# BaratiLab/GAMD

Hardware: AMD Instinct MI355X
Metric: atom-steps/sec (force eval + integrate), 10k-atom LJ box (higher is better)
Workload: dtype f32; 1 GPU; C2: 10 000-atom LJ box, rho*=0.5, L=92.29 A, cutoff 3.0 sigma=10.2 A, fp32, 4 conv layers x 128, random-init weights (seed 0), 1 box per GPU; n_atoms=10000, boxes=1, launch=single process

## Files before the change

gamd_amd/csrc/edge_encode.hip:

```cpp
#include "gamd_common.h"
#include "gamd_internal.h"

namespace {

constexpr int ENC_W1_FLOATS = 4 * 6 * 64 * 4;
constexpr int ENC_LDS_FLOATS = ENC_W1_FLOATS + 2 * GAMD_WFRAG_FLOATS + 5 * 128 + 64;

template <int NFEAT, typename CPtr>
__device__ __forceinline__ void edge_features(const EncArgs& a, CPtr cen, int src, int dst, const float4& ps, const float4& pd,
                                              int half, float (&F)[24]) {
#pragma clang fp contract(off)
    const BoxDims B = gamd_edge_box(a, dst);
    const float rx = gamd_min_image_wrapped(ps.x - pd.x, B.bx, B.hx);
    const float ry = gamd_min_image_wrapped(ps.y - pd.y, B.by, B.hy);
    const float rz = gamd_min_image_wrapped(ps.z - pd.z, B.bz, B.hz);
    const float nrm = sqrtf((rx * rx + ry * ry) + rz * rz);
    const float den = nrm + 1e-8f;
    const float d = (nrm - a.length_mean) / a.length_std;
    F[0] = half ? ry / den : rx / den;
    F[1] = half ? d : rz / den;
    if (a.rbf.uniform) {
        gamd_rbf_chains(d, half, a.gamma * -1.4426950408889634f, a.rbf, F);
    } else {
#pragma unroll
// ... 7 lines not shown
        float flag = 0.f;
        if (a.bond_nbr) {
            const int io = a.perm[dst], jo = a.perm[src];
            const int4 nb = *reinterpret_cast<const int4*>(a.bond_nbr + 4 * (size_t)io);
            flag = (nb.x == jo || nb.y == jo || nb.z == jo || nb.w == jo) ? 1.f : 0.f;
        }
        F[22] = half ? 0.f : flag;
    }
}


__device__ __forceinline__ void gelu_block(const f32x16 (&acc)[4], f32x16 (&X)[4], const GeluCoef& k) {
    __builtin_amdgcn_s_setprio(1);
#pragma unroll
    for (int t = 0; t < 4; ++t)
#pragma unroll
        for (int r = 0; r < 16; r += 2) {
            const gelu_f2 y = gelu_pair(gelu_f2{acc[t][r], acc[t][r + 1]}, k);
            X[t][r] = y[0]; X[t][r + 1] = y[1];
        }
    __builtin_amdgcn_s_setprio(0);
}

template <int NFEAT>
__global__ void __launch_bounds__(512, 2) k_edge_encode(EncArgs a) {
    if (a.devflags[DEVFLAG_FROZEN]) return;
    extern __shared__ __attribute__((aligned(16))) float lds[];
    float* w1 = lds;
    float* w2 = w1 + ENC_W1_FLOATS;
    float* w3 = w2 + GAMD_WFRAG_FLOATS;
    float* vb1 = w3 + GAMD_WFRAG_FLOATS;
    float* vb2 = vb1 + 128;
    float* vb3 = vb2 + 128;
    float* vg = vb3 + 128;
    float* vbeta = vg + 128;
    float* cen = vbeta + 128;

    const int tid = threadIdx.x;
    const GeluCoef gk = gelu_coef();
    for (int i = tid; i < ENC_W1_FLOATS / 4; i += 512) ((f32x4*)w1)[i] = ((const f32x4*)a.w1p)[i];
    for (int i = tid; i < GAMD_WFRAG_FLOATS / 4; i += 512) {
        ((f32x4*)w2)[i] = ((const f32x4*)a.w2p)[i];
        ((f32x4*)w3)[i] = ((const f32x4*)a.w3p)[i];
    }
    if (tid < 128) {
        vb1[tid] = a.b1[tid]; vb2[tid] = a.b2[tid]; vb3[tid] = a.b3[tid];
        vg[tid] = a.ln_g[tid]; vbeta[tid] = a.ln_b[tid];
    }
    if (tid < 40) cen[tid] = a.centers[tid];
    __syncthreads();

    const int lane = tid & 63, wave = tid >> 6, slot = lane & 31, half = lane >> 5;
    long long E = a.counters[CNT_E];
    if (E > a.e_cap) E = a.e_cap;
    const int n_tiles = (int)((E + GAMD_TILE - 1) / GAMD_TILE);
    const int n_units = (n_tiles + 3) / 4;
    int first, end, step;
    gamd_xcd_range(n_units, blockIdx.x, gridDim.x, first, end, step);
    const int n_iter = first < end ? ((end - first + step - 1) / step + 1) / 2 : 0;
    auto tile_of = [&](int it) {
        const int u = first + (2 * it + (wave >> 2)) * step;
        return (it < n_iter && u < end) ? u * 4 + (wave & 3) : n_tiles;
    };

    constexpr int KSTEPS = (NFEAT + 1) / 2;

    int E32 = (int)E;
    auto fetch_idx = [&](int tile, int& src, int& dst) -> bool {
        const int x = tile * GAMD_TILE + gamd_pi(slot);
        const bool ok = tile < n_tiles && x < E32;
        const int xc = ok ? x : 0;
        src = GAMD_CHK_RANGE(a.sticky, a.col[xc], 0, a.zero_row, GAMD_CHK_ENC_SRC); dst = GAMD_CHK_RANGE(a.sticky, a.erow[xc], 0, a.zero_row, GAMD_CHK_ENC_DST);
        return ok;
    };
    int src_c, dst_c;
    {
        const bool ok = fetch_idx(tile_of(0), src_c, dst_c);
        src_c = ok ? src_c : 0; dst_c = ok ? dst_c : 0;
    }
    float4 ps = a.pos_s[src_c], pd = a.pos_s[dst_c];

    for (int it = 0; it < n_iter; ++it) {
        const int tile = tile_of(it);
        int src_n, dst_n;
        const bool ok_n = fetch_idx(tile_of(it + 1), src_n, dst_n);
        if (tile >= n_tiles) { asm volatile("" ::"v"(src_n), "v"(dst_n)); continue; }
        const long long x = (long long)tile * GAMD_TILE + gamd_pi(slot);
        const bool valid = x < E;
        const int src = src_c, dst = dst_c;
        float F[24];
        __builtin_amdgcn_s_setprio(1);
        edge_features<NFEAT>(a, cen, src, dst, ps, pd, half, F);
        asm volatile("" : "+v"(F[0]), "+v"(F[23]));
        __builtin_amdgcn_s_setprio(0);
        if (a.feat_dbg && valid) {
#pragma unroll
            for (int s = 0; s < 24; ++s) a.feat_dbg[x * 48 + 2 * s + half] = F[s];
        }

        f32x16 acc[4], X[4];
        load_bias_chain(vb1, half, acc);
#pragma unroll
        for (int tp = 0; tp < 4; ++tp) {
#pragma unroll
            for (int g = 0; g < 6; ++g) {
                if (4 * g >= KSTEPS) break;
                const f32x4 w = ((const f32x4*)w1)[(tp * 6 + g) * 64 + lane];
#pragma unroll
                for (int j = 0; j < 4; ++j)
                    if (4 * g + j < KSTEPS) acc[tp] = mfma32(w[j], F[4 * g + j], acc[tp]);
            }
        }
        gelu_block(acc, X, gk);
        load_bias_chain(vb2, half, acc);
        gemm128<false>((const f32x4*)w2, lane, X, acc);
        gelu_block(acc, X, gk);
        src_c = ok_n ? src_n : 0; dst_c = ok_n ? dst_n : 0;
        ps = a.pos_s[src_c]; pd = a.pos_s[dst_c];
        load_bias_chain(vb3, half, acc);
        gemm128<false>((const f32x4*)w3, lane, X, acc);
        layernorm_chain_centered(acc, vg, vbeta, half, 1e-5f, a.ln_inv_width);
        if (a.self_loop) {
            if (valid && gamd_is_appended_loop(a, x, src, dst)) {
#pragma unroll
                for (int t = 0; t < 4; ++t)
#pragma unroll
                    for (int r = 0; r < 16; ++r) acc[t][r] = 0.f;
            }
        }
        asm volatile("" ::"v"(ps.x), "v"(ps.y), "v"(ps.z), "v"(ps.w), "v"(pd.x), "v"(pd.y), "v"(pd.z), "v"(pd.w));
        f32x4* out = (f32x4*)a.e_frag + (size_t)tile * 16 * 64;
#pragma unroll
        for (int t = 0; t < 4; ++t)
#pragma unroll
            for (int q = 0; q < 4; ++q) {
                f32x4 v;
#pragma unroll
                for (int j = 0; j < 4; ++j) v[j] = acc[t][q * 4 + j];
                out[(t * 4 + q) * 64 + lane] = v;
            }
    }
}

template <int NFEAT>
__global__ void __launch_bounds__(256) k_edge_encode_small(EncArgs a) {
    if (a.devflags[DEVFLAG_FROZEN]) return;
    __shared__ __attribute__((aligned(16))) float xbuf[32 * GAMD_XLD];
    __shared__ float red[4][64];
    const int lane = threadIdx.x & 63, slot = lane & 31, half = lane >> 5;
    const int quarter = __builtin_amdgcn_readfirstlane(threadIdx.x >> 6);
    long long E = a.counters[CNT_E];
    if (E > a.e_cap) E = a.e_cap;
    const int n_tiles = (int)((E + GAMD_TILE - 1) / GAMD_TILE);
    constexpr int KSTEPS = (NFEAT + 1) / 2;

    for (int tile = blockIdx.x; tile < n_tiles; tile += gridDim.x) {
        const long long x = (long long)tile * GAMD_TILE + gamd_pi(slot);
        const bool valid = x < E;
        const int src = valid ? GAMD_CHK_RANGE(a.sticky, a.col[x], 0, a.zero_row, GAMD_CHK_ENC_SRC) : 0, dst = valid ? GAMD_CHK_RANGE(a.sticky, a.erow[x], 0, a.zero_row, GAMD_CHK_ENC_DST) : 0;
        const float4 ps = a.pos_s[src], pd = a.pos_s[dst];
        f32x4 w1[6];
#pragma unroll
        for (int g = 0; g < 6; ++g) w1[g] = ((const f32x4*)a.w1p)[(quarter * 6 + g) * 64 + lane];
        WQuarter wa, wb;
// ... 37 lines not shown
#pragma unroll
        for (int q = 0; q < 4; ++q) {
            f32x4 o;
#pragma unroll
            for (int j = 0; j < 4; ++j) o[j] = zero_row ? 0.f : fmaf(acc[q * 4 + j] * rstd, g[q * 4 + j], b[q * 4 + j]);
            out[(quarter * 4 + q) * 64 + lane] = o;
        }
    }
}

}

int launch_edge_encode_small(const EncArgs& a, int n_blocks, hipStream_t st) {
    if (a.n_feat == 44) hipLaunchKernelGGL((k_edge_encode_small<44>), dim3(n_blocks), dim3(256), 0, st, a);
    else if (a.n_feat == 45) hipLaunchKernelGGL((k_edge_encode_small<45>), dim3(n_blocks), dim3(256), 0, st, a);
    else return -22;
    GAMD_CHECK_LAUNCH();
    return 0;
}

int launch_edge_encode(const EncArgs& a, int n_blocks, hipStream_t st) {
    const size_t lds = sizeof(float) * ENC_LDS_FLOATS;
    static PerDeviceOnce once;
    if (int e = gamd_allow_dynamic_lds(once, (int)lds, k_edge_encode<44>, k_edge_encode<45>)) return e;
    if (a.n_feat == 44) hipLaunchKernelGGL((k_edge_encode<44>), dim3(n_blocks), dim3(512), lds, st, a);
    else if (a.n_feat == 45) hipLaunchKernelGGL((k_edge_encode<45>), dim3(n_blocks), dim3(512), lds, st, a);
    else return -22;
    GAMD_CHECK_LAUNCH();
    return 0;
}
```

gamd_amd/csrc/gamd_api.hip:

```cpp
#include "../../include/gamd_hip.h"
#include "gamd_common.h"
#include "gamd_internal.h"

#include <algorithm>
#include <cmath>
#include <cstdarg>
#include <cstddef>
#include <cstdio>
#include <cstdlib>
#include <cstring>
#include <deque>
#include <map>
#include <string>
#include <vector>

namespace {

thread_local char g_err[512] = "";

int fail(int code, const char* fmt, ...) {
    va_list ap;
    va_start(ap, fmt);
    vsnprintf(g_err, sizeof(g_err), fmt, ap);
    va_end(ap);
// ... 107 lines not shown
    int Dp = 128, DT = 1;
    int norm_bn = 0;
    bool update_edge = false;
    bool node_f16 = false;
    bool wide_enc = false, wide_conv = false;
    bool l0_hoist = false;
    long long small_tile_limit = 512;
    std::map<std::string, HostTensor> host_w;
    bool finalized = false;
    double scaler_mean = 0.0, scaler_var = 1.0;

    DevBuf wblob;
    std::vector<LayerDev> layers;
    const float *enc_w1p = nullptr, *enc_w2p = nullptr, *enc_w3p = nullptr, *enc_b1 = nullptr, *enc_b2 = nullptr,
                *enc_b3 = nullptr, *enc_lng = nullptr, *enc_lnb = nullptr, *centers = nullptr;
    const float *node_emb = nullptr, *nenc_w = nullptr, *nenc_b = nullptr;
    const float *dec_w1p = nullptr, *dec_b1 = nullptr, *dec_w2 = nullptr, *dec_b2 = nullptr;
    float length_mean = 0.f, length_std = 1.f;
    RbfGrid rbf{};

    DevBuf pos_w, pos_s, cell_of, perm, inv_perm, deg, row_ptr, na_excl, bond_nbr;
    DevBuf hbuf, hn, S, D, P, f_norm, f_den;
    DevBuf l0_h, l0_hn, l0_S, l0_D, l0_P;
    DevBuf cell_cnt, cell_fill, cell_start;
    int ncell_cap = 0;
    long long e_cap = 0;
    long long piece_cap = 0;
    DevBuf col, erow, chunk_piece, chunk_mask, e_frag, partial, feat_dbg, e_emb, e_frag2;
    DevBuf counters, tdbg, tmp_eid, ke_partial, com_partial;
    DevBuf cnt2;
    int cnt_parity = 0;
    long long skin_calls = 0;
    int* cur_counters = nullptr;
    int* counters_host = nullptr;
    float* host_in = nullptr;
    float* host_out = nullptr;
    DevBuf pos_in;
    int* sticky_host = nullptr;
    int* sticky_dev = nullptr;
    hipStream_t init_stream = nullptr;
    DevBuf devflags;
    const float* feat_dev = nullptr;
    const uint8_t* rigid_checked = nullptr;
    MdPending pending;
    Reporter rep;
    bool has_bonds = false;
// ... 356 lines not shown
    ea.devflags = h->devflags.as<int>();
    ea.pos_s = h->pos_s.as<float4>();
    ea.col = h->col.as<int>();
    ea.erow = h->erow.as<int>();
    ea.bond_nbr = h->has_bonds ? h->bond_nbr.as<int>() : nullptr;
    ea.perm = h->perm.as<int>();
    ea.row_ptr = h->row_ptr.as<int>();
    ea.self_loop = na.self_loop;
    ea.zero_row = h->n;
    for (int d = 0; d < 3; ++d) { ea.box[d] = h->box[d]; ea.half[d] = 0.5f * h->box[d]; }
    ea.bx = box_ref(h);
    ea.length_mean = h->length_mean;
    ea.length_std = h->length_std;
    ea.gamma = (float)(1.0 / 0.025);
    ea.ln_inv_width = 1.0f / (float)h->Eh_true;
    ea.ln_n_pad = (float)(h->Eh - h->Eh_true);
    ea.n_feat = h->n_feat;
    ea.n_ksteps = (h->n_feat + 1) / 2;
    ea.centers = h->centers;
    ea.rbf = h->rbf;
    ea.w1p = h->enc_w1p; ea.w2p = h->enc_w2p; ea.w3p = h->enc_w3p;
    ea.b1 = h->enc_b1; ea.b2 = h->enc_b2; ea.b3 = h->enc_b3;
    ea.ln_g = h->enc_lng; ea.ln_b = h->enc_lnb;
    ea.e_format = !h->wide_enc ? 0 : h->cfg.edge_dtype == GAMD_EDGE_F16X3 ? 2 : h->cfg.edge_dtype == GAMD_EDGE_BF16 ? 1 : 0;
    ea.e_frag = h->e_frag.as<float>();
    ea.e_cap = h->e_cap;
    ea.sticky = h->sticky_dev;
    ea.feat_dbg = h->cfg.keep_stages ? h->feat_dbg.as<float>() : nullptr;
    int small_tiles = 0;
    if (h->cfg.edge_dtype == GAMD_EDGE_F32) {
        const long long e_est = el ? el->n + (na.self_loop ? h->n : 0)
                                   : (h->counters_host[CNT_E] > 0 ? (long long)h->counters_host[CNT_E] : (long long)((double)h->e_cap / 1.5));
        const long long tiles = (e_est + GAMD_TILE - 1) / GAMD_TILE;
        if (tiles <= h->small_tile_limit) small_tiles = (int)std::max<long long>(1, std::min<long long>(tiles + tiles / 8 + 1, 4096));
    }
    const bool half_quantum = h->wide_conv && h->cfg.edge_dtype == GAMD_EDGE_F32 && (h->cfg.kernel_select & GAMD_KSEL_FORCE_HALF_QUANTUM) != 0;
    bool tev_full = false;
    auto tev_begin = [&](int kind) -> int {
        if (!h->timing) return 0;
        if (h->tev_used + 2 > h->tev.size()) {
            if (h->tev.size() >= 8 * gamd_handle::EVENT_POOL_CAP) { tev_full = true; return 0; }
            for (int k = 0; k < 256; ++k) { hipEvent_t e; HIP_TRY(hipEventCreate(&e)); h->tev.push_back(e); h->tev_kind.push_back(0); }
        }
        h->tev_kind[h->tev_used] = kind;
        HIP_TRY(hipEventRecord(h->tev[h->tev_used], st));
        return 0;
// ... 36 lines not shown
    no.piece_cap = h->piece_cap;
    no.P_in = h->P.as<float>();
    no.hn_perm = (!h->wide_conv && h->cfg.edge_dtype == GAMD_EDGE_F16X3) ? 1 : 0;
    no.tab16 = (!h->wide_conv && h->cfg.edge_dtype == GAMD_EDGE_BF16) ? 1 : 0;
    no.hn_out = h->hn.as<float>(); no.S_out = h->S.as<float>(); no.D_out = h->D.as<float>(); no.P_out = h->P.as<float>();
    no.dec_w1p = h->dec_w1p; no.dec_b1 = h->dec_b1; no.dec_w2 = h->dec_w2; no.dec_b2 = h->dec_b2;
    no.ln_inv_width = 1.0f / (float)h->H_true;
    no.ln_n_pad = (float)(h->H - h->H_true);
    no.norm_bn = h->norm_bn;
    no.f16x3 = h->node_f16 ? 1 : 0;
    no.scale = (float)std::sqrt(h->scaler_var);
    no.shift = (float)h->scaler_mean;
    no.perm = h->perm.as<int>();
    no.forces_norm = out_norm_dev ? out_norm_dev : h->f_norm.as<float>();
    no.forces = out_denorm_dev;

    const bool l0 = h->skin > 0.f && !el;
    float* const h0 = (l0 && !h->cfg.keep_stages) ? h->l0_h.as<float>() : hptr(0);
    no.mode = 0;
    no.pre = h->layers[0].node;
    no.h_out = h0;
    if (l0) { no.hn_out = h->l0_hn.as<float>(); no.S_out = h->l0_S.as<float>(); no.D_out = h->l0_D.as<float>(); no.P_out = h->l0_P.as<float>(); }
    no.l0_gate = (l0 && l0_reuse) ? 1 : 0;
    if ((r = node(no))) return fail(-1, "node(0) launch failed (%d)", r);
    no.l0_gate = 0;
    no.hn_out = h->hn.as<float>(); no.S_out = h->S.as<float>(); no.D_out = h->D.as<float>(); no.P_out = h->P.as<float>();
    mark("node_first");


    for (int l = 0; l < h->L; ++l) {
        ConvEdgeArgs ca{};
        ca.counters = h->cur_counters;
        ca.devflags = h->devflags.as<int>();
        ca.col = h->col.as<int>(); ca.erow = h->erow.as<int>();
        ca.chunk_piece = h->chunk_piece.as<int>(); ca.chunk_mask = h->chunk_mask.as<unsigned>();
        ca.e_frag = (h->update_edge && l > 0) ? h->e_frag2.as<float>() : h->e_frag.as<float>();
        ca.emb_out = (h->update_edge && l + 1 < h->L) ? h->e_emb.as<float>() : nullptr;
        ca.hn = h->hn.as<float>(); ca.S = h->S.as<float>(); ca.D = h->D.as<float>();
        if (l0 && l == 0) { ca.hn = h->l0_hn.as<float>(); ca.S = h->l0_S.as<float>(); ca.D = h->l0_D.as<float>(); }
        const LayerDev& ld = h->layers[l];
        ca.w1p = ld.w1p; ca.w2p = ld.w2p; ca.w3p = ld.w3p; ca.w4p = ld.w4p; ca.w16p = ld.w16p;
        ca.b1 = ld.b1; ca.b3 = ld.b3; ca.b4 = ld.b4;
        const bool hoist = l == 0 && h->l0_hoist;
        if (hoist) { ca.w3p = ld.w3p_l0; ca.b3 = ld.b3_l0; }
        ca.partial = h->partial.as<float>();
        ca.piece_cap = h->piece_cap;
        ca.sticky = h->sticky_dev;
        ca.e_cap = h->e_cap;
// ... 211 lines not shown
#ifdef GAMD_CHECKED
const char* gamd_version(void) { return "gamd_hip 0.1 (gfx950) checked"; }
#else
const char* gamd_version(void) { return "gamd_hip 0.1 (gfx950)"; }
#endif
const char* gamd_last_error(void) { return g_err; }

int32_t gamd_create(const gamd_config* cfg, gamd_handle** out) {
    if (!cfg || !out) return fail(-22, "null argument");
    if (cfg->n_atoms <= 0) return fail(-22, "n_atoms must be positive");
    if (cfg->n_boxes < 0 || cfg->n_boxes > (1 << 20)) return fail(-22, "n_boxes out of range");
    const int n_boxes = cfg->n_boxes > 1 ? cfg->n_boxes : 1;
    if ((long long)cfg->n_atoms * n_boxes >= (1 << 23) - 1)
        return fail(-22, "n_atoms x n_boxes = %lld: at most %d atoms per handle", (long long)cfg->n_atoms * n_boxes, (1 << 23) - 2);
    if (cfg->n_layers <= 0 || cfg->n_layers > 16) return fail(-22, "n_layers out of range");
    if (!(cfg->cutoff > 0.f)) return fail(-22, "cutoff must be positive");
    if (cfg->edge_dtype != GAMD_EDGE_F32 && cfg->edge_dtype != GAMD_EDGE_BF16 && cfg->edge_dtype != GAMD_EDGE_F16X3)
        return fail(-22, "unknown edge_dtype");
    if (!(cfg->neighbor_skin >= 0.f)) return fail(-22, "neighbor_skin must be >= 0");
    if (cfg->self_loop_mode != GAMD_SELF_LOOP_DGL07_NOOP && cfg->self_loop_mode != GAMD_SELF_LOOP_APPEND_ZERO_FEATURE)
        return fail(-22, "unknown self_loop_mode %d", cfg->self_loop_mode);
    if (cfg->self_loop_mode != GAMD_SELF_LOOP_DGL07_NOOP && cfg->edge_dtype != GAMD_EDGE_F32)
        return fail(-22, "self_loop_mode 1 is built for the fp32 edge dtype only");
    if (cfg->kernel_select & ~(GAMD_KSEL_FORCE_GENERIC_WIDTH | GAMD_KSEL_FORCE_HALF_QUANTUM | GAMD_KSEL_NO_LAYER0_HOIST))
        return fail(-22, "unknown kernel_select bits 0x%x", cfg->kernel_select);
    int ndev = 0;
    if (hipGetDeviceCount(&ndev) != hipSuccess || ndev <= 0)
        return fail(-19, "no HIP device available: libgamd_hip has no CPU fallback");
    if (cfg->device < 0 || cfg->device >= ndev) return fail(-22, "device %d out of range (%d visible)", cfg->device, ndev);
    DeviceGuard guard(cfg->device);
    hipDeviceProp_t prop;
    HIP_TRY(hipGetDeviceProperties(&prop, cfg->device));
    const int H_true = cfg->encoding_size ? cfg->encoding_size : 128, Eh_true = cfg->edge_embedding_dim ? cfg->edge_embedding_dim : 128;
    const int D_true = cfg->hidden_dim ? cfg->hidden_dim : 128;
    if (H_true < 1 || H_true > 256 || Eh_true < 1 || Eh_true > 256)
        return fail(-22, "encoding_size and edge_embedding_dim must be in [1, 256] (got %d, %d)", H_true, Eh_true);
    if (D_true < 1 || D_true > 256) return fail(-22, "hidden_dim must be in [1, 256] (got %d)", D_true);
    const int Dp = D_true <= 128 ? 128 : 256;
    if (Dp > 128 && cfg->edge_dtype != GAMD_EDGE_F32)
        return fail(-22, "hidden_dim above 128 is built for edge_dtype f32 only (got hidden_dim %d)", D_true);
    const int H = H_true <= 128 ? 128 : 256, Eh = Eh_true <= 128 ? 128 : 256;
    const bool exact128 = H_true == 128 && Eh_true == 128 && D_true == 128;
    const bool generic = H != 128 || Eh != 128 || cfg->no_expand_edge;
    if (cfg->edge_dtype != GAMD_EDGE_F32 && H == 256 && (long long)cfg->n_atoms * n_boxes > (1ll << 22) - 2)
        return fail(-22, "bf16 / split-fp16 with encoding_size > 128: at most 2^22 - 2 atoms per handle (32-bit byte offsets into hn)");
    gamd_handle* h = new gamd_handle();
    h->cfg = *cfg;
// ... 450 lines not shown
        LayerDev& d = h->layers[l];
        d.w1p = B + o.w1p; d.w2p = B + o.w2p; d.w3p = B + o.w3p; d.w4p = B + o.w4p;
        d.w16p = (h->wide_conv && h->cfg.edge_dtype == GAMD_EDGE_F32 && DT == 1) ? B + o.w16p : nullptr;
        d.b1 = B + o.b1; d.b3 = B + o.b3; d.b4 = B + o.b4;
        d.node.ln_g = B + o.lng; d.node.ln_b = B + o.lnb;
        if (update_edge) { d.e_ln_g = B + o.elng; d.e_ln_b = B + o.elnb; }
        d.node.wsp = B + o.wsp; d.node.wdp = B + o.wdp; d.node.wpdp = B + o.wpdp;
        d.node.bS = B + o.bS; d.node.bP = B + o.bP;
        d.node.wpep = B + o.wpep; d.node.wphip = B + o.wphip; d.node.bphi = B + o.bphi;
        d.node.c0 = nullptr;
        if (l == 0 && h->l0_hoist) {
            d.w3p_l0 = B + o.w3p_l0; d.b3_l0 = B + o.b3_l0;
            d.node.wpep = B + o.m0; d.node.c0 = B + o.c0;
        }
    }
    h->enc_w1p = B + o_e1; h->enc_w2p = B + o_e2; h->enc_w3p = B + o_e3;
    h->enc_b1 = B + o_eb1; h->enc_b2 = B + o_eb2; h->enc_b3 = B + o_eb3;
    h->enc_lng = B + o_elg; h->enc_lnb = B + o_elb; h->centers = B + o_cen;
    h->dec_w1p = B + o_d1; h->dec_b1 = B + o_db1; h->dec_w2 = B + o_d2; h->dec_b2 = B + o_db2;
    h->node_emb = h->cfg.kind == GAMD_KIND_LJ ? B + o_emb : nullptr;
    h->nenc_w = h->cfg.kind == GAMD_KIND_LJ ? nullptr : B + o_nw;
    h->nenc_b = h->cfg.kind == GAMD_KIND_LJ ? nullptr : B + o_nb;
    h->finalized = true;
    return 0;
}

int32_t gamd_set_scaler(gamd_handle* h, double mean, double var) {
    if (!h) return fail(-22, "null handle");
    if (!(var >= 0.0)) return fail(-22, "scaler variance must be non-negative");
    h->scaler_mean = mean;
    h->scaler_var = var;
    return 0;
}

int32_t gamd_set_bonds(gamd_handle* h, const int32_t* bonds, int64_t n_bonds) {
    if (!h || (!bonds && n_bonds > 0)) return fail(-22, "bad argument to gamd_set_bonds");
    DeviceGuard guard(h->dev);
    InitStream init(h->init_stream);
    std::vector<int> tab((size_t)h->n * 4, -1);
    auto add = [&](int i, int j) -> int {
        for (int k = 0; k < 4; ++k) {
            if (tab[(size_t)i * 4 + k] == j) return 0;
            if (tab[(size_t)i * 4 + k] < 0) { tab[(size_t)i * 4 + k] = j; return 0; }
        }
        return -1;
    };
    for (int box = 0; box < h->n_boxes; ++box)
        for (int64_t b = 0; b < n_bonds; ++b) {
            int i = bonds[2 * b], j = bonds[2 * b + 1];
            if (i < 0 || j < 0 || i >= h->n_per_box || j >= h->n_per_box)
                return fail(-22, "bond %lld references atom out of range", (long long)b);
            i += box * h->n_per_box; j += box * h->n_per_box;
            if (add(i, j) || add(j, i)) return fail(-22, "more than 4 bonded partners for one atom is not supported");
        }
    if (h->bond_nbr.ensure(sizeof(int) * tab.size(), false)) return fail(-12, "bond table allocation failed");
    HIP_TRY(init_upload(h->bond_nbr.p, tab.data(), sizeof(int) * tab.size()));
    h->has_bonds = n_bonds > 0;
    return 0;
}

int32_t gamd_set_node_features(gamd_handle* h, const float* feat_dev) {
    if (!h) return fail(-22, "null handle");
    if (feat_dev && h->cfg.kind != GAMD_KIND_WATER) return fail(-22, "node features belong to the water models (the LJ model has node_emb)");
    h->feat_dev = feat_dev;
    return 0;
}

int32_t gamd_get_device_flags(gamd_handle* h, int32_t flags[4]) {
    if (!h || !flags) return fail(-22, "null argument");
    flags[0] = h->sticky_host[STICKY_NONFINITE] ? 1 : 0;
    flags[1] = flags[2] = flags[3] = 0;
    h->sticky_host[STICKY_NONFINITE] = 0;
    return 0;
}

int32_t gamd_build_neighbors(gamd_handle* h, const float* pos_dev, const uint8_t* species_dev, const float* box, void* stream) {
    int r;
    if ((r = check_ready(h))) return r;
    if (!pos_dev || !box) return fail(-22, "null argument");
    DeviceGuard guard(h->dev);
    InitStream init((hipStream_t)stream);
    hipStream_t st = (hipStream_t)stream;
    for (int attempt = 0; attempt < 4; ++attempt) {
        if ((r = set_box(h, box, st))) return r;
        h->cur_counters = h->counters.as<int>();
        NbrArgs na = nbr_args(h, pos_dev, species_dev);
        h->cand_valid = false;
// ... 490 lines not shown
```

gamd_amd/csrc/gamd_internal.h:

```cpp
#pragma once
#include <hip/hip_runtime.h>
#include <stdint.h>
#include <atomic>
#include "gamd_common.h"

enum { CNT_E = 0, CNT_PIECES = 1, CNT_OVERFLOW = 2, CNT_TILES = 3, CNT_REBUILD = 4, CNT_NCAND = 5,
       CNT_CAND_MAX = 6,
       CNT_COUNT = 8 };
enum { STICKY_EDGE_OVERFLOW = 0, STICKY_CAND_OVERFLOW = 1, STICKY_REBUILDS = 2, STICKY_NCAND = 3,
       STICKY_NONFINITE = 4,
       STICKY_CHECK_CODE = 5, STICKY_CHECK_VALUE = 6, STICKY_CHECK_LINE = 7,
       STICKY_COUNT = 8 };
enum { GAMD_CHK_CELL = 101, GAMD_CHK_CAND = 102, GAMD_CHK_EDGE_POS = 103, GAMD_CHK_PERM = 104, GAMD_CHK_ENC_SRC = 111, GAMD_CHK_ENC_DST = 112,
       GAMD_CHK_CONV_SRC = 121, GAMD_CHK_CONV_DST = 122, GAMD_CHK_PIECE = 123, GAMD_CHK_NODE_PIECES = 131, GAMD_CHK_INJECTED = 199 };
#ifdef GAMD_CHECKED
template <typename T>
__device__ __forceinline__ T gamd_chk_range(int* sticky, T v, long long lo, long long hi, int code, int line) {
    if ((long long)v >= lo && (long long)v <= hi) return v;
    if (sticky && sticky[STICKY_CHECK_CODE] == 0) {
        sticky[STICKY_CHECK_VALUE] = (int)v;
        sticky[STICKY_CHECK_LINE] = line;
        __threadfence_system();
        sticky[STICKY_CHECK_CODE] = code;
    }
// ... 101 lines not shown
    const int* erow;
    const int* bond_nbr;
    const int* perm;
    const int* row_ptr;
    int self_loop;
    int zero_row;
    float box[3], half[3];
    BoxRef bx;
    float length_mean, length_std, gamma;
    float ln_inv_width, ln_n_pad;
    int n_feat;
    int n_ksteps;
    const float* centers;
    RbfGrid rbf;
    const float* w1p;
    const float* w2p;
    const float* w3p;
    const float* b1; const float* b2; const float* b3;
    const float* ln_g; const float* ln_b;
    float* e_frag;
    long long e_cap;
    float* feat_dbg;
    int* sticky;
    int e_format;
};
__device__ __forceinline__ bool gamd_is_appended_loop(const EncArgs& a, long long x, int src, int dst) {
    if (!a.self_loop || src == a.zero_row) return false;
    const long long row_end = a.row_ptr[dst + 1];
    return x == row_end - 1 || (x + 1 < row_end && a.col[x + 1] == a.zero_row);
}

__device__ __forceinline__ BoxDims gamd_edge_box(const EncArgs& a, int dst) {
    return gamd_box_dims(a.bx, a.box, a.half, a.bx.n_boxes > 1 ? gamd_box_of(a.bx, dst) : 0);
}
int launch_edge_encode(const EncArgs& a, int n_blocks, hipStream_t st);
int launch_edge_encode_small(const EncArgs& a, int n_blocks, hipStream_t st);
int launch_edge_encode_bf16(const EncArgs& a, int n_blocks, hipStream_t st);
int launch_edge_encode_f16x3(const EncArgs& a, int n_blocks, hipStream_t st);
int launch_edge_encode_wide(const EncArgs& a, int eht, int n_blocks, hipStream_t st);
int launch_edge_encode_wide_d(const EncArgs& a, int eht, int dt, int n_blocks, hipStream_t st);

struct ConvEdgeArgs {
    const int* counters;
    const int* devflags;
    const int* col;
    const int* erow;
// ... 35 lines not shown
    const float* ln_g; const float* ln_b;
    float ln_inv_width, ln_n_pad;
    float* e_frag_out;
};
int launch_edge_update(const EdgeUpdateArgs& a, int ht, int n_blocks, hipStream_t st);

struct NodeLayerW {
    const float* ln_g; const float* ln_b;
    const float* wsp; const float* wdp; const float* wpdp;
    const float* bS;
    const float* bP;
    const float* wpep;
    const float* c0;
    const float* wphip;
    const float* bphi;
};
struct NodeArgs {
    const int* counters;
    const int* devflags;
    int* sticky;
    int n;
    int mode;
    int l0_gate;
    const float4* pos_s;
    const float* node_emb;
    const float* enc_w; const float* enc_b;
    const int* row_ptr; const int* na_excl; const int* deg;
    const int* col;
    const float* partial;
    long long piece_cap;
    const float* h_in;
    const float* P_in;
    NodeLayerW post;
    NodeLayerW pre;
    const float* dec_w1p; const float* dec_b1; const float* dec_w2; const float* dec_b2;
    float scale, shift;
    float ln_inv_width, ln_n_pad;
    int norm_bn;
    int f16x3;
    const int* perm;
    float* h_out;
    float* hn_out; float* S_out; float* D_out; float* P_out;
    int hn_perm;
    int tab16;
    float* forces_norm;
    float* forces;
// ... 92 lines not shown
```

gamd_amd/csrc/node.hip:

```cpp
#include "gamd_common.h"
#include "gamd_internal.h"

namespace {

typedef _Float16 nf16x8 __attribute__((ext_vector_type(8)));
typedef _Float16 nf16x2 __attribute__((ext_vector_type(2)));
typedef float nf32x2 __attribute__((ext_vector_type(2)));

constexpr int NT = 16;
constexpr int XLD = 136;

__device__ __forceinline__ f32x4 mfma16(float a, float b, f32x4 c) {
    return __builtin_amdgcn_mfma_f32_16x16x4f32(a, b, c, 0, 0, 0);
}

struct WHalf { f32x4 w[8]; };
__device__ __forceinline__ void load_whalf(const float* __restrict__ Wp, int w, int lane, int half, WHalf& h) {
    const f32x4* W = reinterpret_cast<const f32x4*>(Wp) + (size_t)w * 16 * 64 + lane;
#pragma unroll
    for (int o = 0; o < 2; ++o)
#pragma unroll
        for (int b = 0; b < 4; ++b) h.w[o * 4 + b] = W[(o * 8 + 4 * half + b) * 64];
}

// ... 76 lines not shown
    const nf16x2 lo = __builtin_convertvector(nf32x2{v[0], v[1]}, nf16x2), hi = __builtin_convertvector(nf32x2{v[2], v[3]}, nf16x2);
    return nf16x4{lo[0], lo[1], hi[0], hi[1]};
}
__device__ __forceinline__ void store16_h(_Float16* __restrict__ row, int w, int g, const f32x4 (&v)[2]) {
    *reinterpret_cast<nf16x4*>(row + 32 * w + 4 * g) = cvt16x4(v[0]);
    *reinterpret_cast<nf16x4*>(row + 32 * w + 16 + 4 * g) = cvt16x4(v[1]);
}
__device__ __forceinline__ void store16_tab(_Float16* __restrict__ row, int w, int g, const f32x4 (&v)[2]) {
    *reinterpret_cast<nf16x4*>(row + 32 * w + 8 * (g & 1) + 4 * (g >> 1)) = cvt16x4(v[0]);
    *reinterpret_cast<nf16x4*>(row + 32 * w + 16 + 8 * (g & 1) + 4 * (g >> 1)) = cvt16x4(v[1]);
}

__device__ __forceinline__ float group_sum(float v) {
    v += __shfl_xor(v, 16, 64);
    return v + __shfl_xor(v, 32, 64);
}

template <bool F16>
__global__ void __launch_bounds__(256, 3) k_node(NodeArgs a) {
    __shared__ __attribute__((aligned(16))) float xbuf[NT * XLD];
    __shared__ float obuf[4][NT][3];
    __shared__ float red[2][4][NT];

    if (a.counters[CNT_OVERFLOW] || a.devflags[DEVFLAG_FROZEN]) return;
    if (a.mode == 0 && a.l0_gate && a.counters[CNT_REBUILD] == 0) return;

    const int lane = threadIdx.x & 63, la = lane & 15, g = lane >> 4;
    const int w = __builtin_amdgcn_readfirstlane(threadIdx.x >> 6);
    const int atom_raw = blockIdx.x * NT + la;
    const bool valid = atom_raw < a.n;
    const int atom = valid ? atom_raw : a.n - 1;
    const size_t row = (size_t)atom * GAMD_H;

#ifdef GAMD_PROFILING
    long long tm[16] = {0, 0, 0, 0, 0, 0, 0, 0, 0, 0, 0, 0, 0, 0, 0, 0};
#define NMARK(I) do { if (a.tdbg) tm[I] = (long long)__builtin_readcyclecounter(); } while (0)
#else
#define NMARK(I) do { } while (0)
#endif
    NMARK(0);
    f32x4 XB[8];
    XSplit XS;
#define GEMM16(NEXT, W, NXT) do { if constexpr (F16) gemm16<NEXT, true>(W, NXT, wn, XS, mine, w, lane); \
                                  else gemm16<NEXT, false>(W, NXT, wn, XB, mine, w, lane); } while (0)
#define SPLIT16() do { if constexpr (F16) split16(XB, XS); } while (0)
    f32x4 mine[2];
    WHalf wn;
// ... 203 lines not shown
```

gamd_amd/csrc/wide.hip:

```cpp
#include "gamd_common.h"
#include "gamd_bf16.h"
#include "gamd_f16x3.h"
#include "gamd_internal.h"
#include "gamd_wide.h"

namespace {

constexpr int WIDE_ENC_W1_FLOATS = 4 * 6 * 64 * 4;

__device__ __forceinline__ void wide_barrier() {
    asm volatile("s_waitcnt vmcnt(0) lgkmcnt(0)" ::: "memory");
    __builtin_amdgcn_s_barrier();
    asm volatile("" ::: "memory");
}

template <int EHT> struct EncWaves { static constexpr int value = EHT == 2 ? 4 : 8; };

template <int NFEAT, int EHT, bool LP = false>
__global__ void __launch_bounds__(64 * EncWaves<EHT>::value) k_edge_encode_wide(EncArgs a) {
    if (a.devflags[DEVFLAG_FROZEN]) return;
    static_assert(EHT == 1 || EHT == 2, "edge embedding width 128 or 256");
    constexpr int EH = 128 * EHT;
    constexpr int NW = EncWaves<EHT>::value, NT = 64 * NW;
    constexpr bool EXPAND = NFEAT >= 44;
// ... 375 lines not shown
    for (int i = 0; i < 8; ++i) { o.w[i] = W[i * 64]; o.w[8 + i] = W[2048 + i * 64]; }
}
__device__ __forceinline__ void wq_gemm_f16(const WQ& wq, const f32x16 (&X)[4], f32x16& acc) {
#pragma unroll
    for (int t = 0; t < 4; ++t)
#pragma unroll
        for (int u = 0; u < 2; ++u) {
            f16x8 xh, xl;
            gamd_split8(X[t], u, xh, xl);
            const f16x8 wh = __builtin_bit_cast(f16x8, wq.w[t * 2 + u]), wl = __builtin_bit_cast(f16x8, wq.w[8 + t * 2 + u]);
            acc = mfma_f16(wh, xl, acc);
            acc = mfma_f16(wl, xh, acc);
            acc = mfma_f16(wh, xh, acc);
        }
}
template <int HT, bool F16 = false>
__global__ void __launch_bounds__(256) k_node_wide(NodeArgs a) {
    constexpr int H = 128 * HT;
    constexpr int XLDW = H + 4;
    __shared__ __attribute__((aligned(16))) float xbuf[32 * XLDW];
    __shared__ float obuf[4][32][3];
    __shared__ float red[2][4][32];

    if (a.counters[CNT_OVERFLOW] || a.devflags[DEVFLAG_FROZEN]) return;
    if (a.mode == 0 && a.l0_gate && a.counters[CNT_REBUILD] == 0) return;

    const int lane = threadIdx.x & 63, slot = lane & 31, half = lane >> 5;
    const int quarter = __builtin_amdgcn_readfirstlane(threadIdx.x >> 6);
    const int atom_raw = blockIdx.x * GAMD_TILE + slot;
    const bool valid = atom_raw < a.n;
    const int atom = valid ? atom_raw : a.n - 1;
    const size_t rowH = (size_t)atom * H, rowD = (size_t)atom * 128;

    f32x16 X[HT][4];
    f32x16 mine[HT];
    WQ wqa, wqb;
    constexpr size_t BLK = GAMD_WFRAG_FLOATS;
    auto wptr = [&](int st) -> const float* {
        if (st < HT) return a.post.wpep + (size_t)st * BLK;
        if (st < 2 * HT) return a.post.wphip + (size_t)(st - HT) * BLK;
        const int i = st - 2 * HT;
        if (a.mode == 2) return i < HT ? a.dec_w1p + (size_t)i * BLK : nullptr;
        if (i < HT) return a.pre.wsp + (size_t)i * BLK;
        if (i < 2 * HT) return a.pre.wdp + (size_t)(i - HT) * BLK;
        return i < 3 * HT ? a.pre.wpdp + (size_t)(i - 2 * HT) * BLK : nullptr;
    };
    auto step = [&](int st, const f32x16 (&Xb)[4], f32x16& acc) {
// ... 230 lines not shown
```

gamd_amd/csrc/wide_d.hip:

```cpp
#include "gamd_common.h"
#include "gamd_internal.h"
#include "gamd_wide.h"

namespace {

constexpr int ENC_W1_BLOCK_FLOATS = 4 * 6 * 64 * 4;

__device__ __forceinline__ void wd_barrier() {
    asm volatile("s_waitcnt vmcnt(0) lgkmcnt(0)" ::: "memory");
    __builtin_amdgcn_s_barrier();
    asm volatile("" ::: "memory");
}

template <int NP>
struct BlockRing {
    const float* blocks;
    float* lds;
    int wave;
    unsigned lane16;
    unsigned g = 0;
    int blk = 0;
    __device__ __forceinline__ void prime() { gamd_stage_weight_raw_contig<4>(blocks, lds, wave, lane16); }
    __device__ __forceinline__ const f32x4* begin() {
        const int nb = (blk + 1 == NP) ? 0 : blk + 1;
// ... 319 lines not shown
                                    for (int k = 1; k < 16; ++k) v = (r == k) ? U[tp][k] : v;
                                    a.partial[(size_t)p * H + 128 * ob + 32 * tp + slot] = v;
                                }
                                ++p;
                            }
                        }
                    }
                }
                ring.end();
            }
        }
    }
}


template <int HT, int DT>
__global__ void __launch_bounds__(256) k_node_wide_d(NodeArgs a) {
    constexpr int H = 128 * HT, DP = 128 * DT, NB = HT * DT;
    constexpr int XLDW = 128 * (HT > DT ? HT : DT) + 4;
    __shared__ __attribute__((aligned(16))) float xbuf[32 * XLDW];
    __shared__ float obuf[4][32][3];
    __shared__ float red[2][4][32];

    if (a.counters[CNT_OVERFLOW] || a.devflags[DEVFLAG_FROZEN]) return;
    if (a.mode == 0 && a.l0_gate && a.counters[CNT_REBUILD] == 0) return;

    const int lane = threadIdx.x & 63, slot = lane & 31, half = lane >> 5;
    const int quarter = __builtin_amdgcn_readfirstlane(threadIdx.x >> 6);
    const int atom_raw = blockIdx.x * GAMD_TILE + slot;
    const bool valid = atom_raw < a.n;
    const int atom = valid ? atom_raw : a.n - 1;
    const size_t rowH = (size_t)atom * H, rowD = (size_t)atom * DP;

    f32x16 XH[HT][4];
    f32x16 mine[HT];
    WQ wqa, wqb;
    constexpr size_t BLK = GAMD_WFRAG_FLOATS;
    auto wptr = [&](int st) -> const float* {
        if (st < NB) return a.post.wpep + (size_t)st * BLK;
        if (st < 2 * NB) return a.post.wphip + (size_t)(st - NB) * BLK;
        const int i = st - 2 * NB;
        if (a.mode == 2) return i < NB ? a.dec_w1p + (size_t)i * BLK : nullptr;
        if (i < NB) return a.pre.wsp + (size_t)i * BLK;
        if (i < 2 * NB) return a.pre.wdp + (size_t)(i - NB) * BLK;
        return i < 3 * NB ? a.pre.wpdp + (size_t)(i - 2 * NB) * BLK : nullptr;
    };
    auto step = [&](int st, const f32x16 (&Xb)[4], f32x16& acc) {
// ... 233 lines not shown
```

gamd_amd/engine.py:

```python
from __future__ import annotations

import ctypes as C
from typing import Dict, Optional, Sequence, Tuple, Union

import numpy as np
import torch

from . import _lib
from ._lib import GamdReportParams, GamdConfig, GamdMdParams, GamdNhcParams, check
from .weights import ModelConfig, infer_config, validate_state_dict

ArrayLike = Union[np.ndarray, torch.Tensor]

KIND = {"lj": 0, "water": 1, "dynbox": 1}
FLAVOUR = {"jaxmd": 0, "torch": 1}
SELF_LOOP = {"dgl07_noop": 0, "append_zero_feature_loops": 1}
KSEL_FORCE_GENERIC_WIDTH = 1
KSEL_NO_LAYER0_HOIST = 4


def _box3(box) -> np.ndarray:
    b = np.asarray(box, dtype=np.float64).reshape(-1)
    if b.size == 1:
        b = np.repeat(b, 3)
    if b.size != 3:
        raise ValueError("box must be a scalar or 3 values")
    return b.astype(np.float32)


def _boxes(box, n_boxes: int) -> np.ndarray:
    b = np.asarray(box, dtype=np.float64)
    if b.ndim == 0 or b.size == 1 or (b.ndim == 1 and b.size == 3):
        return np.tile(_box3(b), (n_boxes, 1))
    if b.ndim == 2 and b.shape == (n_boxes, 3):
        return b.astype(np.float32)
    if (b.ndim == 1 and b.size == n_boxes) or (b.ndim == 2 and b.shape == (n_boxes, 1)):
        return np.repeat(b.reshape(-1).astype(np.float32)[:, None], 3, axis=1)
    raise ValueError(f"box must be a scalar, 3 values, [{n_boxes}, 1] or [{n_boxes}, 3] ({n_boxes} boxes)")


class RunReport:
# ... 447 lines not shown
```

include/gamd_hip.h:

```cpp
#ifndef GAMD_HIP_H
#define GAMD_HIP_H

#include <stdint.h>
#include <stddef.h>

#ifdef __cplusplus
extern "C" {
#endif

typedef struct gamd_handle gamd_handle;

enum { GAMD_EDGE_F32 = 0, GAMD_EDGE_BF16 = 1, GAMD_EDGE_F16X3 = 2 };

enum { GAMD_KIND_LJ = 0, GAMD_KIND_WATER = 1 };
enum { GAMD_NBR_JAXMD = 0, GAMD_NBR_TORCH = 1 };

typedef struct gamd_config {
    int32_t n_atoms;
    int32_t kind;
    int32_t n_layers;
    int32_t use_bond;
    int32_t nbr_flavour;
    int32_t device;
    float cutoff;
    float box[3];
    int64_t edge_capacity;
    int32_t keep_stages;
    int32_t edge_dtype;
    int32_t encoding_size;
    int32_t edge_embedding_dim;
    int32_t hidden_dim;
    int32_t no_expand_edge;
    float neighbor_skin;
    int32_t self_loop_mode;
    int32_t kernel_select;
    int32_t small_tile_limit;
    int32_t n_boxes;
} gamd_config;
enum { GAMD_SELF_LOOP_DGL07_NOOP = 0, GAMD_SELF_LOOP_APPEND_ZERO_FEATURE = 1 };
enum { GAMD_KSEL_FORCE_GENERIC_WIDTH = 1, GAMD_KSEL_FORCE_HALF_QUANTUM = 2, GAMD_KSEL_NO_LAYER0_HOIST = 4 };

const char* gamd_version(void);
const char* gamd_last_error(void);

int32_t gamd_create(const gamd_config* cfg, gamd_handle** out);
int32_t gamd_destroy(gamd_handle* h);

int32_t gamd_load_weight(gamd_handle* h, const char* name, const float* data, const int64_t* shape, int32_t ndim);
int32_t gamd_finalize_weights(gamd_handle* h);

int32_t gamd_set_scaler(gamd_handle* h, double mean, double var);

int32_t gamd_set_bonds(gamd_handle* h, const int32_t* bonds, int64_t n_bonds);

int32_t gamd_forces_async(gamd_handle* h, const float* pos_dev, const uint8_t* species_dev, const float* box,
                          float* out_norm_dev, float* out_denorm_dev, void* stream);

int32_t gamd_set_node_features(gamd_handle* h, const float* feat_dev);

int32_t gamd_sync_status(gamd_handle* h, void* stream);

int32_t gamd_get_device_flags(gamd_handle* h, int32_t flags[4]);

// ... 93 lines not shown
```

Baseline: 3.371 million atom-steps/s.

## Overlap encoder weight staging with first tile; cache constant layer-0 node table

```diff
diff --git a/gamd_amd/csrc/edge_encode.hip b/gamd_amd/csrc/edge_encode.hip
--- a/gamd_amd/csrc/edge_encode.hip
+++ b/gamd_amd/csrc/edge_encode.hip
@@ -1,3 +1,4 @@
+#include <type_traits>
 #include "gamd_common.h"
 #include "gamd_internal.h"
 
@@ -53,7 +54,14 @@
     __builtin_amdgcn_s_setprio(0);
 }
 
-template <int NFEAT>
+template <int N>
+__device__ __forceinline__ void weights_landed() {
+    asm volatile("s_waitcnt vmcnt(%0) lgkmcnt(0)" ::"n"(N) : "memory");
+    __builtin_amdgcn_s_barrier();
+    asm volatile("" ::: "memory");
+}
+
+template <int NFEAT, bool OVERLAP>
 __global__ void __launch_bounds__(512, 2) k_edge_encode(EncArgs a) {
     if (a.devflags[DEVFLAG_FROZEN]) return;
     extern __shared__ __attribute__((aligned(16))) float lds[];
@@ -69,19 +77,8 @@
 
     const int tid = threadIdx.x;
     const GeluCoef gk = gelu_coef();
-    for (int i = tid; i < ENC_W1_FLOATS / 4; i += 512) ((f32x4*)w1)[i] = ((const f32x4*)a.w1p)[i];
-    for (int i = tid; i < GAMD_WFRAG_FLOATS / 4; i += 512) {
-        ((f32x4*)w2)[i] = ((const f32x4*)a.w2p)[i];
-        ((f32x4*)w3)[i] = ((const f32x4*)a.w3p)[i];
-    }
-    if (tid < 128) {
-        vb1[tid] = a.b1[tid]; vb2[tid] = a.b2[tid]; vb3[tid] = a.b3[tid];
-        vg[tid] = a.ln_g[tid]; vbeta[tid] = a.ln_b[tid];
-    }
-    if (tid < 40) cen[tid] = a.centers[tid];
-    __syncthreads();
-
-    const int lane = tid & 63, wave = tid >> 6, slot = lane & 31, half = lane >> 5;
+    const int lane = tid & 63, slot = lane & 31, half = lane >> 5;
+    const int wave = __builtin_amdgcn_readfirstlane(tid >> 6);
     long long E = a.counters[CNT_E];
     if (E > a.e_cap) E = a.e_cap;
     const int n_tiles = (int)((E + GAMD_TILE - 1) / GAMD_TILE);
@@ -104,18 +101,53 @@
         src = GAMD_CHK_RANGE(a.sticky, a.col[xc], 0, a.zero_row, GAMD_CHK_ENC_SRC); dst = GAMD_CHK_RANGE(a.sticky, a.erow[xc], 0, a.zero_row, GAMD_CHK_ENC_DST);
         return ok;
     };
+    auto stage_small = [&]() {
+        for (int i = tid; i < ENC_W1_FLOATS / 4; i += 512) ((f32x4*)w1)[i] = ((const f32x4*)a.w1p)[i];
+        if (tid < 128) {
+            vb1[tid] = a.b1[tid]; vb2[tid] = a.b2[tid]; vb3[tid] = a.b3[tid];
+            vg[tid] = a.ln_g[tid]; vbeta[tid] = a.ln_b[tid];
+        }
+        if (tid < 40) cen[tid] = a.centers[tid];
+    };
+    constexpr bool overlap = OVERLAP;
+    if (overlap && n_iter == 0) return;
     int src_c, dst_c;
-    {
+    float4 ps, pd;
+    if (overlap) {
         const bool ok = fetch_idx(tile_of(0), src_c, dst_c);
         src_c = ok ? src_c : 0; dst_c = ok ? dst_c : 0;
+        ps = a.pos_s[src_c]; pd = a.pos_s[dst_c];
+        stage_small();
+        asm volatile("s_waitcnt vmcnt(0)" ::"v"(ps.x), "v"(ps.y), "v"(ps.z), "v"(ps.w), "v"(pd.x), "v"(pd.y), "v"(pd.z), "v"(pd.w) : "memory");
+        gamd_stage_weight_raw_contig<8>(a.w2p, w2, wave, (unsigned)lane * 16u);
+        gamd_stage_weight_raw_contig<8>(a.w3p, w3, wave, (unsigned)lane * 16u);
+        asm volatile("s_waitcnt lgkmcnt(0)" ::: "memory");
+        __builtin_amdgcn_s_barrier();
+        asm volatile("" ::: "memory");
+    } else {
+        stage_small();
+        for (int i = tid; i < GAMD_WFRAG_FLOATS / 4; i += 512) {
+            ((f32x4*)w2)[i] = ((const f32x4*)a.w2p)[i];
+            ((f32x4*)w3)[i] = ((const f32x4*)a.w3p)[i];
+        }
+        __syncthreads();
+        const bool ok = fetch_idx(tile_of(0), src_c, dst_c);
+        src_c = ok ? src_c : 0; dst_c = ok ? dst_c : 0;
+        ps = a.pos_s[src_c]; pd = a.pos_s[dst_c];
     }
-    float4 ps = a.pos_s[src_c], pd = a.pos_s[dst_c];
-
-    for (int it = 0; it < n_iter; ++it) {
+
+    auto iteration = [&](int it, auto first_tag) __attribute__((always_inline)) {
+        constexpr bool landing = OVERLAP && decltype(first_tag)::value;
+        int half_v = half;
+        asm volatile("" : "+v"(half_v));
         const int tile = tile_of(it);
         int src_n, dst_n;
         const bool ok_n = fetch_idx(tile_of(it + 1), src_n, dst_n);
-        if (tile >= n_tiles) { asm volatile("" ::"v"(src_n), "v"(dst_n)); continue; }
+        if (tile >= n_tiles) {
+            asm volatile("" ::"v"(src_n), "v"(dst_n));
+            if (landing) { weights_landed<0>(); weights_landed<0>(); }
+            return;
+        }
         const long long x = (long long)tile * GAMD_TILE + gamd_pi(slot);
         const bool valid = x < E;
         const int src = src_c, dst = dst_c;
@@ -130,7 +162,7 @@
         }
 
         f32x16 acc[4], X[4];
-        load_bias_chain(vb1, half, acc);
+        load_bias_chain(vb1, half_v, acc);
 #pragma unroll
         for (int tp = 0; tp < 4; ++tp) {
 #pragma unroll
@@ -143,14 +175,16 @@
             }
         }
         gelu_block(acc, X, gk);
-        load_bias_chain(vb2, half, acc);
+        if (landing) weights_landed<8>();
+        load_bias_chain(vb2, half_v, acc);
         gemm128<false>((const f32x4*)w2, lane, X, acc);
         gelu_block(acc, X, gk);
+        if (landing) weights_landed<0>();
         src_c = ok_n ? src_n : 0; dst_c = ok_n ? dst_n : 0;
         ps = a.pos_s[src_c]; pd = a.pos_s[dst_c];
-        load_bias_chain(vb3, half, acc);
+        load_bias_chain(vb3, half_v, acc);
         gemm128<false>((const f32x4*)w3, lane, X, acc);
-        layernorm_chain_centered(acc, vg, vbeta, half, 1e-5f, a.ln_inv_width);
+        layernorm_chain_centered(acc, vg, vbeta, half_v, 1e-5f, a.ln_inv_width);
         if (a.self_loop) {
             if (valid && gamd_is_appended_loop(a, x, src, dst)) {
 #pragma unroll
@@ -170,7 +204,10 @@
                 for (int j = 0; j < 4; ++j) v[j] = acc[t][q * 4 + j];
                 out[(t * 4 + q) * 64 + lane] = v;
             }
-    }
+    };
+    int it0 = 0;
+    if (OVERLAP) { iteration(0, std::true_type{}); it0 = 1; }
+    for (int it = it0; it < n_iter; ++it) iteration(it, std::false_type{});
 }
 
 template <int NFEAT>
@@ -254,9 +291,11 @@
 int launch_edge_encode(const EncArgs& a, int n_blocks, hipStream_t st) {
     const size_t lds = sizeof(float) * ENC_LDS_FLOATS;
     static PerDeviceOnce once;
-    if (int e = gamd_allow_dynamic_lds(once, (int)lds, k_edge_encode<44>, k_edge_encode<45>)) return e;
-    if (a.n_feat == 44) hipLaunchKernelGGL((k_edge_encode<44>), dim3(n_blocks), dim3(512), lds, st, a);
-    else if (a.n_feat == 45) hipLaunchKernelGGL((k_edge_encode<45>), dim3(n_blocks), dim3(512), lds, st, a);
+    if (int e = gamd_allow_dynamic_lds(once, (int)lds, k_edge_encode<44, true>, k_edge_encode<45, true>, k_edge_encode<44, false>, k_edge_encode<45, false>)) return e;
+    if (a.n_feat == 44 && a.stage_overlap) hipLaunchKernelGGL((k_edge_encode<44, true>), dim3(n_blocks), dim3(512), lds, st, a);
+    else if (a.n_feat == 44) hipLaunchKernelGGL((k_edge_encode<44, false>), dim3(n_blocks), dim3(512), lds, st, a);
+    else if (a.n_feat == 45 && a.stage_overlap) hipLaunchKernelGGL((k_edge_encode<45, true>), dim3(n_blocks), dim3(512), lds, st, a);
+    else if (a.n_feat == 45) hipLaunchKernelGGL((k_edge_encode<45, false>), dim3(n_blocks), dim3(512), lds, st, a);
     else return -22;
     GAMD_CHECK_LAUNCH();
     return 0;
diff --git a/gamd_amd/csrc/gamd_api.hip b/gamd_amd/csrc/gamd_api.hip
--- a/gamd_amd/csrc/gamd_api.hip
+++ b/gamd_amd/csrc/gamd_api.hip
@@ -153,6 +153,7 @@
     DevBuf pos_w, pos_s, cell_of, perm, inv_perm, deg, row_ptr, na_excl, bond_nbr;
     DevBuf hbuf, hn, S, D, P, f_norm, f_den;
     DevBuf l0_h, l0_hn, l0_S, l0_D, l0_P;
+    bool l0_written = false;
     DevBuf cell_cnt, cell_fill, cell_start;
     int ncell_cap = 0;
     long long e_cap = 0;
@@ -555,6 +556,7 @@
     ea.w1p = h->enc_w1p; ea.w2p = h->enc_w2p; ea.w3p = h->enc_w3p;
     ea.b1 = h->enc_b1; ea.b2 = h->enc_b2; ea.b3 = h->enc_b3;
     ea.ln_g = h->enc_lng; ea.ln_b = h->enc_lnb;
+    ea.stage_overlap = (h->cfg.kernel_select & GAMD_KSEL_NO_ENC_OVERLAP) ? 0 : 1;
     ea.e_format = !h->wide_enc ? 0 : h->cfg.edge_dtype == GAMD_EDGE_F16X3 ? 2 : h->cfg.edge_dtype == GAMD_EDGE_BF16 ? 1 : 0;
     ea.e_frag = h->e_frag.as<float>();
     ea.e_cap = h->e_cap;
@@ -637,8 +639,18 @@
     no.h_out = h0;
     if (l0) { no.hn_out = h->l0_hn.as<float>(); no.S_out = h->l0_S.as<float>(); no.D_out = h->l0_D.as<float>(); no.P_out = h->l0_P.as<float>(); }
     no.l0_gate = (l0 && l0_reuse) ? 1 : 0;
-    if ((r = node(no))) return fail(-1, "node(0) launch failed (%d)", r);
+    bool l0_cache = l0 && !h->cfg.keep_stages && h->node_emb && !h->feat_dev && !(h->cfg.kernel_select & GAMD_KSEL_NO_L0_TABLE_CACHE);
+    if (l0_cache && !h->l0_written) {
+        hipStreamCaptureStatus cs = hipStreamCaptureStatusNone;
+        if (hipStreamIsCapturing(st, &cs) != hipSuccess || cs != hipStreamCaptureStatusNone) l0_cache = false;
+    }
+    if (!(l0_cache && h->l0_written)) {
+        if (l0_cache) { no.l0_gate = 0; no.l0_const = 1; }
+        if ((r = node(no))) return fail(-1, "node(0) launch failed (%d)", r);
+        if (l0_cache) h->l0_written = true;
+    }
     no.l0_gate = 0;
+    no.l0_const = 0;
     no.hn_out = h->hn.as<float>(); no.S_out = h->S.as<float>(); no.D_out = h->D.as<float>(); no.P_out = h->P.as<float>();
     mark("node_first");
 
@@ -896,7 +908,8 @@
         return fail(-22, "unknown self_loop_mode %d", cfg->self_loop_mode);
     if (cfg->self_loop_mode != GAMD_SELF_LOOP_DGL07_NOOP && cfg->edge_dtype != GAMD_EDGE_F32)
         return fail(-22, "self_loop_mode 1 is built for the fp32 edge dtype only");
-    if (cfg->kernel_select & ~(GAMD_KSEL_FORCE_GENERIC_WIDTH | GAMD_KSEL_FORCE_HALF_QUANTUM | GAMD_KSEL_NO_LAYER0_HOIST))
+    if (cfg->kernel_select & ~(GAMD_KSEL_FORCE_GENERIC_WIDTH | GAMD_KSEL_FORCE_HALF_QUANTUM | GAMD_KSEL_NO_LAYER0_HOIST |
+                               GAMD_KSEL_NO_L0_TABLE_CACHE | GAMD_KSEL_NO_ENC_OVERLAP))
         return fail(-22, "unknown kernel_select bits 0x%x", cfg->kernel_select);
     int ndev = 0;
     if (hipGetDeviceCount(&ndev) != hipSuccess || ndev <= 0)
@@ -1393,6 +1406,7 @@
     h->nenc_w = h->cfg.kind == GAMD_KIND_LJ ? nullptr : B + o_nw;
     h->nenc_b = h->cfg.kind == GAMD_KIND_LJ ? nullptr : B + o_nb;
     h->finalized = true;
+    h->l0_written = false;
     return 0;
 }
 
@@ -1434,6 +1448,7 @@
     if (!h) return fail(-22, "null handle");
     if (feat_dev && h->cfg.kind != GAMD_KIND_WATER) return fail(-22, "node features belong to the water models (the LJ model has node_emb)");
     h->feat_dev = feat_dev;
+    h->l0_written = false;
     return 0;
 }
 
diff --git a/gamd_amd/csrc/gamd_internal.h b/gamd_amd/csrc/gamd_internal.h
--- a/gamd_amd/csrc/gamd_internal.h
+++ b/gamd_amd/csrc/gamd_internal.h
@@ -147,6 +147,7 @@
     long long e_cap;
     float* feat_dbg;
     int* sticky;
+    int stage_overlap;
     int e_format;
 };
 __device__ __forceinline__ bool gamd_is_appended_loop(const EncArgs& a, long long x, int src, int dst) {
@@ -228,6 +229,7 @@
     int n;
     int mode;
     int l0_gate;
+    int l0_const;
     const float4* pos_s;
     const float* node_emb;
     const float* enc_w; const float* enc_b;
diff --git a/gamd_amd/csrc/node.hip b/gamd_amd/csrc/node.hip
--- a/gamd_amd/csrc/node.hip
+++ b/gamd_amd/csrc/node.hip
@@ -122,7 +122,7 @@
     __shared__ float obuf[4][NT][3];
     __shared__ float red[2][4][NT];
 
-    if (a.counters[CNT_OVERFLOW] || a.devflags[DEVFLAG_FROZEN]) return;
+    if (!(a.mode == 0 && a.l0_const) && (a.counters[CNT_OVERFLOW] || a.devflags[DEVFLAG_FROZEN])) return;
     if (a.mode == 0 && a.l0_gate && a.counters[CNT_REBUILD] == 0) return;
 
     const int lane = threadIdx.x & 63, la = lane & 15, g = lane >> 4;
diff --git a/gamd_amd/csrc/wide.hip b/gamd_amd/csrc/wide.hip
--- a/gamd_amd/csrc/wide.hip
+++ b/gamd_amd/csrc/wide.hip
@@ -421,7 +421,7 @@
     __shared__ float obuf[4][32][3];
     __shared__ float red[2][4][32];
 
-    if (a.counters[CNT_OVERFLOW] || a.devflags[DEVFLAG_FROZEN]) return;
+    if (!(a.mode == 0 && a.l0_const) && (a.counters[CNT_OVERFLOW] || a.devflags[DEVFLAG_FROZEN])) return;
     if (a.mode == 0 && a.l0_gate && a.counters[CNT_REBUILD] == 0) return;
 
     const int lane = threadIdx.x & 63, slot = lane & 31, half = lane >> 5;
diff --git a/gamd_amd/csrc/wide_d.hip b/gamd_amd/csrc/wide_d.hip
--- a/gamd_amd/csrc/wide_d.hip
+++ b/gamd_amd/csrc/wide_d.hip
@@ -365,7 +365,7 @@
     __shared__ float obuf[4][32][3];
     __shared__ float red[2][4][32];
 
-    if (a.counters[CNT_OVERFLOW] || a.devflags[DEVFLAG_FROZEN]) return;
+    if (!(a.mode == 0 && a.l0_const) && (a.counters[CNT_OVERFLOW] || a.devflags[DEVFLAG_FROZEN])) return;
     if (a.mode == 0 && a.l0_gate && a.counters[CNT_REBUILD] == 0) return;
 
     const int lane = threadIdx.x & 63, slot = lane & 31, half = lane >> 5;
diff --git a/gamd_amd/engine.py b/gamd_amd/engine.py
--- a/gamd_amd/engine.py
+++ b/gamd_amd/engine.py
@@ -17,6 +17,8 @@
 SELF_LOOP = {"dgl07_noop": 0, "append_zero_feature_loops": 1}
 KSEL_FORCE_GENERIC_WIDTH = 1
 KSEL_NO_LAYER0_HOIST = 4
+KSEL_NO_L0_TABLE_CACHE = 8
+KSEL_NO_ENC_OVERLAP = 32
 
 
 def _box3(box) -> np.ndarray:
diff --git a/include/gamd_hip.h b/include/gamd_hip.h
--- a/include/gamd_hip.h
+++ b/include/gamd_hip.h
@@ -38,7 +38,8 @@
     int32_t n_boxes;
 } gamd_config;
 enum { GAMD_SELF_LOOP_DGL07_NOOP = 0, GAMD_SELF_LOOP_APPEND_ZERO_FEATURE = 1 };
-enum { GAMD_KSEL_FORCE_GENERIC_WIDTH = 1, GAMD_KSEL_FORCE_HALF_QUANTUM = 2, GAMD_KSEL_NO_LAYER0_HOIST = 4 };
+enum { GAMD_KSEL_FORCE_GENERIC_WIDTH = 1, GAMD_KSEL_FORCE_HALF_QUANTUM = 2, GAMD_KSEL_NO_LAYER0_HOIST = 4,
+       GAMD_KSEL_NO_L0_TABLE_CACHE = 8, GAMD_KSEL_NO_ENC_OVERLAP = 32 };
 
 const char* gamd_version(void);
 const char* gamd_last_error(void);
```

After: 3.369 million atom-steps/s. About the same (-0.1%).
